# AIRI-Institute/HairFastGAN

Hardware: AMD Instinct MI355X
Metric: stylegan2_generator_fwd_1024_images_per_sec (higher is better)
Workload: dtype f32 tensors + f32 accumulate; conv products as 3 fp16 MFMAs on (hi,lo)-split operands (fp32-class); 1 GPU; StyleGAN2 1024^2 generator forward (range 0->8), random W+, fresh noise per layer, HIP modulated-conv + upfirdn2d kernels (BASELINE.json configs[1]); batch_per_gpu=8, global_batch=8, parallelism=replica x1, weights=synthetic closed-form (oracle/synth.py), conv_precision=f16x3

## Files before the change

### hairfastgan_amd/csrc/convh.hip

```cpp
#define HF_WANT_F16_SPLIT
#include <type_traits>

#include "conv_common.h"

using namespace hf_detail;

#ifdef HF_H_TRACE
__device__ unsigned long long hf_trace_buf[8 * 512];
#define HF_TRACE_POINT(id)                                                                    \
  do {                                                                                         \
    if (blockIdx.x == 0 && blockIdx.y == 0 && lane == 0 && wave < 8 && trace_n < 510) {                    \
      hf_trace_buf[wave * 512 + trace_n++] = ((unsigned long long)(id) << 56) | (__builtin_readcyclecounter() & 0xffffffffffffffULL); \
    }                                                                                          \
  } while (0)
extern "C" int hf_debug_read_trace(unsigned long long *host, int n) {
  return (int)hipMemcpyFromSymbol(host, HIP_SYMBOL(hf_trace_buf), sizeof(unsigned long long) * n);
}
#else
#define HF_TRACE_POINT(id) ((void)0)
#endif

namespace {

typedef _Float16 half8 __attribute__((ext_vector_type(8)));
// ... 2 lines not shown
template <int NR, int NM>
__device__ __forceinline__ void hf_interleave() {
#pragma unroll
  for (int k = 0; k < NR; ++k) {
    __builtin_amdgcn_sched_group_barrier(0x008, 1, 0);
    __builtin_amdgcn_sched_group_barrier(0x100, 1, 0);
  }
  if constexpr (NM > NR) __builtin_amdgcn_sched_group_barrier(0x008, NM - NR, 0);
}

template <int PT, bool UP, int TWMAX, bool FUSE = false>
constexpr int halo_pixels_max() {
  constexpr int h = UP ? 1 : 2;
  constexpr int narrow = (PT / 32 + h) * (32 + h), wide = (PT / TWMAX + h) * (TWMAX + h);
  constexpr int main_tile = wide > narrow ? wide : narrow;
  constexpr int rim = PT >= 512 ? 4 : 2;
  constexpr int rim_tile = (rim + 1) * (PT / rim + 1);
  return (UP && !FUSE && rim_tile > main_tile) ? rim_tile : main_tile;
}

template <bool UP>
__host__ __device__ constexpr int tap_at(int i) {
  return !UP ? i : (i == 2 ? 3 : i == 3 ? 4 : i == 4 ? 2 : i);
}
template <bool UP>
__host__ __device__ constexpr int tap_group(int i) {
  return !UP ? i : (i < 4 ? 0 : i < 6 ? 1 : i < 8 ? 2 : 3);
}
template <bool UP>
__host__ __device__ constexpr int group_first(int g) {
  return !UP ? g : (g == 0 ? 0 : g == 1 ? 4 : g == 2 ? 6 : g == 3 ? 8 : 9);
}

template <int NTERMS, int CT_TILES, int PG, int WAVES_CO, int WAVES_PX, bool UP, int TWMAX, bool FUSE>
struct HShape {
  static constexpr int NW = WAVES_CO * WAVES_PX;
  static constexpr int NT = 64 * NW;
  static constexpr int CT = 32 * CT_TILES * WAVES_CO;
  static constexpr int PT = 32 * PG * WAVES_PX;
  static constexpr int XSLOTS = (PG == 1) ? 4 : 6;
  using Stage = StageLayout<NTERMS, CT, halo_pixels_max<PT, UP, TWMAX, FUSE>(), FUSE ? NW * XSLOTS * 64 : 0>;
  static constexpr int TABLE_FLOATS = 2 * 3 * CT;
  static size_t lds_bytes(int cin, bool rgb) {
    return Stage::stage_bytes + (Stage::cin_table_floats(cin) + (rgb ? 2 : 1) * TABLE_FLOATS) * sizeof(float);
  }
};

template <int NTERMS, int CT_TILES, int PG, int WAVES_CO, int WAVES_PX, bool MOD, bool UP, int TWMAX, bool PRE, bool FUSE = false>
__global__ __launch_bounds__(64 * WAVES_CO * WAVES_PX, (WAVES_CO * WAVES_PX >= 16 ? 4 : 2)) void conv_mfma_h(const ConvParams P,
                                                                          const _Float16 *__restrict__ wth,
                                                                          const _Float16 *__restrict__ wtl) {
  using S = HShape<NTERMS, CT_TILES, PG, WAVES_CO, WAVES_PX, UP, TWMAX, FUSE>;
  using L = typename S::Stage;
  constexpr int NW = S::NW, NT = S::NT, CT = S::CT, PT = S::PT, XSLOTS = S::XSLOTS;
  constexpr int NPH = UP ? 4 : 1;
  constexpr int HALO = UP ? 1 : 2;
  constexpr int NPIX = L::NPIX, NPART = L::NPART, W_UNITS = L::W_UNITS, X_UNITS = L::X_UNITS, BUF_UNITS = L::BUF_UNITS;
  constexpr int N_WPIECE = NPART * W_UNITS / 64;
  constexpr bool PP = PRE && NW == 8;
  constexpr int ND = (N_WPIECE + NW - 1) / NW;
  constexpr int DMA_PER_STEP = PRE ? 1 : (ND + 2) / 3;
  constexpr int XE = (X_UNITS + NT - 1) / NT;
  static_assert(W_UNITS % 64 == 0, "weight part must be whole 1 KiB pieces");
  static_assert(!FUSE || (UP && CT_TILES == 1 && WAVES_CO == 1 && TWMAX == 32), "FUSE: 32 co x (PG*WAVES_PX rows of 32 positions)");
  static_assert(!FUSE || BUF_UNITS * 16 >= NW * XSLOTS * 64 * 16, "FUSE: the exchange of one channel quad must fit a stage buffer");
  static_assert(!PRE || (ND <= 9 && XE <= 8), "PRE issue schedule: one weight DMA per tap-step, activations in odd steps (or every step)");

  HF_DYN_LDS;
  half8 *lds = reinterpret_cast<half8 *>(hf_dyn_lds);
  constexpr int OFF_WL = L::OFF_WL, OFF_XH = L::OFF_XH, OFF_XL = L::OFF_XL;

  const int tid = threadIdx.x;
  const int lane = tid & 63;
  const int wave = tid >> 6;
  const int li = lane & 31;
  const int lh = lane >> 5;
  const int wave_co = (wave / WAVES_PX) * (32 * CT_TILES);
  const int wave_pg = (wave % WAVES_PX) * PG;
  const int blk_x = P.swap_xy ? (int)blockIdx.y : (int)blockIdx.x, blk_y = P.swap_xy ? (int)blockIdx.x : (int)blockIdx.y;
  const int grid_x = P.swap_xy ? (int)gridDim.y : (int)gridDim.x, grid_y = P.swap_xy ? (int)gridDim.x : (int)gridDim.y;
  const int co0 = blk_y * CT;

  const long long plane = (long long)P.h * P.w;
  const int iplane = (int)plane;
  const int nchunks = P.cin / KH;
  float *sl_base = reinterpret_cast<float *>(lds + 2 * BUF_UNITS);
  float *ep_base = sl_base + L::cin_table_floats(P.cin);
  float *rgbw_base = ep_base + S::TABLE_FLOATS;

  struct Tile {
    int gi, b0, ty0, tx0;
  };
  const TileGeom G0 = P.g[0], G1 = P.g[1], G2 = P.g[2];
  auto geom = [&](int gi) {
    TileGeom G;
#define HF_PICK(f) G.f = gi == 0 ? G0.f : (gi == 1 ? G1.f : G2.f)
    HF_PICK(y0); HF_PICK(x0); HF_PICK(dh); HF_PICK(dw); HF_PICK(lg_tw); HF_PICK(lg_th); HF_PICK(lg_nb);
    HF_PICK(tiles_x); HF_PICK(tiles_y); HF_PICK(tiles_b); HF_PICK(first_block);
#undef HF_PICK
    return G;
  };
  auto locate = [&](int t) {
    Tile T;
    T.gi = 0;
    if (P.n_geom > 1 && t >= G1.first_block) T.gi = 1;
    if (P.n_geom > 2 && t >= G2.first_block) T.gi = 2;
    const TileGeom G = geom(T.gi);
    int r = t - G.first_block;
    const int tx = r % G.tiles_x;
    r /= G.tiles_x;
    const int ty = r % G.tiles_y;
    T.b0 = r / G.tiles_y;
    T.ty0 = G.y0 + (ty << G.lg_th);
    T.tx0 = G.x0 + (tx << G.lg_tw);
    if (FUSE) {
      T.ty0 = ty * ((1 << G.lg_th) - 2) - 1;
      T.tx0 = tx * ((1 << G.lg_tw) - 2) - 1;
    }
    return T;
  };
  constexpr int NSRC = XE;
  auto locate_items = [&](const Tile &T, int (&src)[NSRC]) {
    const TileGeom G = geom(T.gi);
    const int wp = (1 << G.lg_tw) + HALO, xs = ((1 << G.lg_th) + HALO) * wp;
#pragma unroll
    for (int e = 0; e < XE; ++e) {
      const int i = tid + e * NT;
      const int kg = i / NPIX, pix = i - kg * NPIX;
      src[e] = -2;
      if (i < X_UNITS && pix < xs) {
        const int hy = pix / wp, hx = pix - hy * wp;
        const int ys = T.ty0 + hy - 1, xc = T.tx0 + hx - 1;
        src[e] = (ys >= 0 && ys < P.h && xc >= 0 && xc < P.w) ? ys * P.w + xc : -1;
      }
    }
  };
  const float w_unscale = *reinterpret_cast<const float *>(wth + 9LL * P.cin * P.cout);
  const bool fast_ep = !UP && HF_STD_STYLED_TAIL(P);
  const float ep_fold = (FUSE || fast_ep) ? P.scale : 1.0f;
  auto load_s = [&](int b, int slot) {
    float *dst = sl_base + slot * P.cin;
    if (MOD)
      for (int i = tid; i < P.cin; i += NT) dst[i] = P.s[(long long)b * P.s_bstride + i];
    float *ep = ep_base + slot * 3 * CT;
    for (int i = tid; i < CT; i += NT) {
      ep[i] = (P.d ? P.d[(long long)b * P.d_bstride + co0 + i] : 1.0f) * w_unscale * ep_fold;
      ep[CT + i] = P.bias ? P.bias[co0 + i] * ep_fold : 0.0f;
      ep[2 * CT + i] = ((!UP || FUSE) && P.oh && P.s_next) ? P.s_next[(long long)b * P.cout + co0 + i] : 1.0f;
    }
    if (!UP && P.rgb_out) {
      float *rw = rgbw_base + slot * 3 * CT;
      for (int i = tid; i < CT; i += NT) {
        const float sv = P.rgb_s[(long long)b * P.cout + co0 + i];
#pragma unroll
        for (int c = 0; c < 3; ++c) rw[c * CT + i] = P.rgb_w[(co0 + i) * 3 + c] * sv;
      }
    }
  };

  int e_src[XE];
  const float *xb;
  int sl_off;
  int sl_slot = 0;

  const unsigned lds_addr0 = hf_lds_addr(lds);
  auto dma_piece = [&](int i, int chunk, int bufsel) {
    const int pc = wave + i * NW;
    if (wave < NW && pc < N_WPIECE) {
      const int part = pc / (W_UNITS / 64), q = pc % (W_UNITS / 64);
      const int u = q * 64 + lane;
      const int row = u / CT, col = u % CT;
      int off = (row * P.cout + co0 + col) * 16;
      HF_OPAQUE_I32(off);
      const _Float16 *src = (part ? wtl : wth) + (long long)chunk * 18 * P.cout * 8;
      hf_glds16_raw_s(src, (unsigned)off, lds_addr0 + (unsigned)(bufsel * BUF_UNITS + part * W_UNITS + q * 64) * 16u);
    }
  };

  const char *xh_b = nullptr, *xl_b = nullptr;
  auto dma_x = [&](int e, int chunk, int bufsel) {
    const int i = tid + e * NT;
    const int kg = i / NPIX;
    const bool inside = e_src[e] >= 0;
    int off = inside ? (kg * iplane + e_src[e]) * 16 : 0;
    HF_OPAQUE_I32(off);
    const long long cofs = (long long)chunk * 2 * plane * 16;
    const unsigned dst = lds_addr0 + (unsigned)(bufsel * BUF_UNITS + OFF_XH + (i - lane)) * 16u;
    hf_glds16_raw_s_if(inside, xh_b + cofs, (unsigned)off, dst);
    if (NTERMS == 3) hf_glds16_raw_s_if(inside, xl_b + cofs, (unsigned)off, dst + (unsigned)X_UNITS * 16u);
    if (e_src[e] == -1) {
      half8 z;
#pragma unroll
      for (int k = 0; k < 8; ++k) z[k] = (_Float16)0.0f;
      half8 *buf = lds + bufsel * BUF_UNITS;
      buf[OFF_XH + i] = z;
      if (NTERMS == 3) buf[OFF_XL + i] = z;
    }
  };

  float xr[XE][8];
  auto load_item = [&](int e, int chunk) {
    const char *xc = reinterpret_cast<const char *>(xb + (long long)chunk * KH * plane);
    const int kg = (tid + e * NT) / NPIX;
    int off = (e_src[e] >= 0) ? kg * 8 * iplane + e_src[e] : 0;
    HF_OPAQUE_I32(off);
#pragma unroll
    for (int k = 0; k < 8; ++k)
      xr[e][k] = *reinterpret_cast<const float *>(xc + (unsigned)((off + k * iplane) * 4));
  };
  auto convert_item = [&](int e, int chunk, half8 *buf) {
    if (e_src[e] == -2) return;
    const int i = tid + e * NT;
    const int kg = i / NPIX;
    half8 hi, lo;
    bool ovf = false;
#pragma unroll
    for (int k = 0; k < 8; ++k) {
      float v = (e_src[e] >= 0) ? xr[e][k] : 0.0f;
      if (MOD) v *= sl_base[sl_off + chunk * KH + kg * 8 + k];
      _Float16 hv, lv;
      hf_split_f16(v, hv, lv, ovf);
      hi[k] = hv;
      lo[k] = lv;
    }
    hf_note_overflow(ovf);
    buf[OFF_XH + i] = hi;
    if (NTERMS == 3) buf[OFF_XL + i] = lo;
  };

  f32x16 acc[NPH][CT_TILES][PG];
  auto zero_acc = [&]() {
#pragma unroll
    for (int ph = 0; ph < NPH; ++ph)
#pragma unroll
      for (int ct = 0; ct < CT_TILES; ++ct)
#pragma unroll
        for (int g = 0; g < PG; ++g)
#pragma unroll
          for (int r = 0; r < 16; ++r) acc[ph][ct][g][r] = 0.0f;
  };
  zero_acc();

  int t_cur = blk_x;
  Tile cur = locate(t_cur);
  locate_items(cur, e_src);
  xb = P.x + (long long)cur.b0 * P.cin * plane;
  if (PRE) {
    xh_b = static_cast<const char *>(P.xh) + (long long)cur.b0 * (P.cin / 8) * plane * 16;
    xl_b = static_cast<const char *>(P.xl) + (long long)cur.b0 * (P.cin / 8) * plane * 16;
  }
  sl_off = 0;
  load_s(cur.b0, 0);
  int ep_slot = 0;
  __syncthreads();
#pragma unroll
  for (int i = 0; i < ND; ++i) dma_piece(i, 0, 0);
  if (PRE) {
#pragma unroll
    for (int e = 0; e < XE; ++e) dma_x(e, 0, 0);
  } else {
#pragma unroll
    for (int e = 0; e < XE; ++e) load_item(e, 0);
#pragma unroll
    for (int e = 0; e < XE; ++e) convert_item(e, 0, lds);
  }
  hf_barrier_keep_young<0>();

  int trace_n = 0;
  (void)trace_n;
  const float nw_ = (!UP && P.noise) ? P.noise_w[0] : 0.0f;
  auto epilogue = [&](const TileGeom &G, const Tile &T, int slot, const float (&nz)[PG]) {
    int co_w = wave_co, li_o = li, lh_o = lh;
    HF_OPAQUE_I32(co_w);
    HF_OPAQUE_I32(li_o);
    HF_OPAQUE_I32(lh_o);
    const int tw = 1 << G.lg_tw, th = 1 << G.lg_th;
    const float *ep = ep_base + slot * 3 * CT;
    const unsigned oplane4 = (unsigned)(P.out_h * P.out_w) * 4u;
    char *ob0 = reinterpret_cast<char *>(P.out + ((long long)T.b0 * P.cout + co0) * ((long long)P.out_h * P.out_w));
#pragma unroll
    for (int g = 0; g < PG; ++g) {
      const int p = (wave_pg + g) * 32 + li_o;
      const int Y = T.ty0 + ((p >> G.lg_tw) & (th - 1)), X = T.tx0 + (p & (tw - 1));
      const bool pv = (Y < G.y0 + G.dh) && (X < G.x0 + G.dw);
      const float nzv = nw_ * nz[g];
      float rgb[3] = {0.0f, 0.0f, 0.0f};
      if (pv) {
      const unsigned pix4 = UP ? (unsigned)(2 * Y * P.out_w + 2 * X) * 4u : (unsigned)(Y * P.out_w + X) * 4u;
#pragma unroll
      for (int ct = 0; ct < CT_TILES; ++ct)
#pragma unroll
        for (int q = 0; q < 4; ++q) {
          const int c4 = co_w + ct * 32 + 8 * q + 4 * lh_o;
          const float4 dm = *reinterpret_cast<const float4 *>(ep + c4);
          const float4 bs = *reinterpret_cast<const float4 *>(ep + CT + c4);
          const float dmv[4] = {dm.x, dm.y, dm.z, dm.w}, bsv[4] = {bs.x, bs.y, bs.z, bs.w};
          unsigned off = (unsigned)c4 * oplane4 + pix4;
#pragma unroll
          for (int k = 0; k < 4; ++k, off += oplane4) {
// ... 135 lines not shown
            hf_half4 h4, l4;
            bool ovf = false;
            hf_split4_f16(vs, h4, l4, ovf);
            if (pvg[g]) {
              ovf_tile = ovf_tile || ovf;
              const unsigned off = cofs16 + pix16[g];
              *reinterpret_cast<hf_half4 *>(oh_t + off) = h4;
              if (ol_t) *reinterpret_cast<hf_half4 *>(ol_t + off) = l4;
            }
          }
          if (RGB) {
#pragma unroll
            for (int c = 0; c < 3; ++c)
              rgb[g][c] = fmaf(v[3], wv[c].w, fmaf(v[2], wv[c].z, fmaf(v[1], wv[c].y, fmaf(v[0], wv[c].x, rgb[g][c]))));
          }
        }
      }
    if (RGB) {
      const int slabs = grid_y * WAVES_CO, slab = blk_y * WAVES_CO + wave / WAVES_PX;
#pragma unroll
      for (int g = 0; g < PG; ++g)
#pragma unroll
        for (int c = 0; c < 3; ++c) {
          const float sum = rgb[g][c] + __shfl_xor(rgb[g][c], 32, 64);
          if (pvg[g] && lh_o == 0)
            P.rgb_out[(((long long)T.b0 * slabs + slab) * 3 + c) * ((long long)P.out_h * P.out_w) + (long long)Yg[g] * P.out_w + Xg[g]] = sum;
        }
    }
    if (SPLIT) hf_note_overflow(ovf_tile);
  };

  const float kxf[4] = {P.blur_kx[0], P.blur_kx[1], P.blur_kx[2], P.blur_kx[3]};
  const float kyf[4] = {P.blur_ky[0], P.blur_ky[1], P.blur_ky[2], P.blur_ky[3]};
  auto epilogue_fused = [&](auto SPLIT_T, const Tile &T, int slot, const float (&nz)[PG][4], int freebuf) {
    constexpr bool SPLIT = decltype(SPLIT_T)::value;
    bool ovf_tile = false;
    int li_o = li, lh_o = lh;
    HF_OPAQUE_I32(li_o);
    HF_OPAQUE_I32(lh_o);
    const float *ep = ep_base + slot * 3 * CT;
    const int wv = wave;
    float *xch = reinterpret_cast<float *>(lds + freebuf * BUF_UNITS);
    const int row0 = wv * PG;
    const int Y0 = T.ty0 + row0, X = T.tx0 + li_o;
    const float nw_f = (P.noise ? P.noise_w[0] : 0.0f) * P.scale;
    const long long oplane = (long long)(2 * P.h) * (2 * P.w);
    const int pix00 = (2 * Y0) * (2 * P.w) + 2 * X;
    const bool colv = li_o >= 1 && li_o <= 30 && X >= 0 && X < P.w;
    char *oh_b = SPLIT ? static_cast<char *>(P.oh) + ((long long)T.b0 * (P.cout >> 3) + (co0 >> 3)) * oplane * 16 : nullptr;
    char *ol_b = SPLIT ? static_cast<char *>(P.ol) + ((long long)T.b0 * (P.cout >> 3) + (co0 >> 3)) * oplane * 16 : nullptr;
    float *of_b = SPLIT ? nullptr : P.out + ((long long)T.b0 * P.cout + co0) * oplane;
#pragma unroll
    for (int q = 0; q < 4; ++q) {
      __builtin_amdgcn_sched_barrier(0);
      float H[4][PG][4];
#pragma unroll
      for (int pr = 0; pr < 2; ++pr)
#pragma unroll
        for (int g = 0; g < PG; ++g)
#pragma unroll
          for (int k = 0; k < 4; ++k) {
            const float t0 = acc[2 * pr][0][g][4 * q + k], t1 = acc[2 * pr + 1][0][g][4 * q + k];
            const float l1 = hf_lane_up(t1), r0 = hf_lane_down(t0), r1 = hf_lane_down(t1);
            H[2 * pr][g][k] = fmaf(kxf[3], r0, fmaf(kxf[2], t1, fmaf(kxf[1], t0, kxf[0] * l1)));
            H[2 * pr + 1][g][k] = fmaf(kxf[3], r1, fmaf(kxf[2], r0, fmaf(kxf[1], t1, kxf[0] * t0)));
          }
      HF_TRACE_POINT(30);
      float4 *xq = reinterpret_cast<float4 *>(xch);
      float4 *mine = xq + (wv * XSLOTS) * 64 + lane;
#pragma unroll
      for (int ph = 0; ph < 4; ++ph) mine[ph * 64] = make_float4(H[ph][0][0], H[ph][0][1], H[ph][0][2], H[ph][0][3]);
      if (PG > 1) {
#pragma unroll
        for (int pc = 0; pc < 2; ++pc)
          mine[(4 + pc) * 64] = make_float4(H[2 + pc][PG - 1][0], H[2 + pc][PG - 1][1], H[2 + pc][PG - 1][2], H[2 + pc][PG - 1][3]);
      }
      HF_TRACE_POINT(31);
      hf_barrier_lds();
      HF_TRACE_POINT(32);
      const float4 *above = xq + (max(wv - 1, 0) * XSLOTS) * 64 + lane, *below = xq + (min(wv + 1, NW - 1) * XSLOTS) * 64 + lane;
      constexpr int ABOVE_P1 = (PG == 1) ? 2 : 4;
      const int c4 = 8 * q + 4 * lh_o;
#pragma unroll
      for (int g = 0; g < PG; ++g) {
        const int rr = row0 + g, Y = Y0 + g;
        const bool pv = colv && rr >= 1 && rr <= PT / 32 - 2 && Y >= 0 && Y < P.h;
#pragma unroll
        for (int a = 0; a < 2; ++a) {
          typedef unsigned u32x2 __attribute__((ext_vector_type(2)));
          typedef unsigned u32x4 __attribute__((ext_vector_type(4)));
          u32x2 hq[2], lq[2];
          bool ovf_a = false;
#pragma unroll
          for (int pc = 0; pc < 2; ++pc) {
            float hm1[4], h2[4], h3[4];
            if (g == 0 && a == 0) {
              const float4 u = above[(ABOVE_P1 + pc) * 64];
              hm1[0] = u.x; hm1[1] = u.y; hm1[2] = u.z; hm1[3] = u.w;
            }
            if (g == PG - 1) {
              const float4 d0 = below[pc * 64];
              h2[0] = d0.x; h2[1] = d0.y; h2[2] = d0.z; h2[3] = d0.w;
              if (a == 1) {
                const float4 d1 = below[(2 + pc) * 64];
                h3[0] = d1.x; h3[1] = d1.y; h3[2] = d1.z; h3[3] = d1.w;
              }
            }
            const float4 dm = *reinterpret_cast<const float4 *>(ep + c4), bs = *reinterpret_cast<const float4 *>(ep + CT + c4);
            const float dmv[4] = {dm.x, dm.y, dm.z, dm.w}, bsv[4] = {bs.x, bs.y, bs.z, bs.w};
            float v[4];
#pragma unroll
            for (int k = 0; k < 4; ++k) {
              const float h_m1 = (g == 0) ? hm1[k] : H[2 + pc][g == 0 ? 0 : g - 1][k];
// ... 65 lines not shown
#pragma unroll
    for (int g = 0; g < PG; ++g) {
      const int p = (wave_pg + g) * 32 + li;
      const int po = ((p >> G.lg_tw) & (th - 1)) * wp + (p & (tw - 1));
#pragma unroll
      for (int r = 0; r < NROW; ++r) pixrow[g][r] = po + r * wp;
    }
    float nzr[PG];
    float nzf[PG][4];
#pragma unroll
    for (int g = 0; g < PG; ++g) {
      nzr[g] = 0.0f;
#pragma unroll
      for (int k = 0; k < 4; ++k) nzf[g][k] = 0.0f;
    }
    HF_TRACE_POINT(7);
    const int t_next = t_cur + grid_x;
    const bool has_next = t_next < P.n_tiles;
    Tile nxt = cur;
    int nxt_sl_off = sl_off;
    if (has_next) {
      nxt = locate(t_next);
      if (nxt.b0 != cur.b0) {
        hf_barrier_lds();
        sl_slot ^= 1;
        nxt_sl_off = sl_slot * P.cin;
        load_s(nxt.b0, sl_slot);
      }
    }
    HF_TRACE_POINT(8);

    for (int c = 0; c < nchunks; ++c, ++stage) {
      const int cb = stage & 1;
      half8 *buf = lds + cb * BUF_UNITS, *nbuf = lds + (cb ^ 1) * BUF_UNITS;
      const bool last = c + 1 == nchunks;
      const bool more1 = !last || has_next;
      const int cpf = last ? 0 : c + 1;
      if (last && has_next) {
        locate_items(nxt, e_src);
        xb = P.x + (long long)nxt.b0 * P.cin * plane;
        if (PRE) {
          xh_b = static_cast<const char *>(P.xh) + (long long)nxt.b0 * (P.cin / 8) * plane * 16;
          xl_b = static_cast<const char *>(P.xl) + (long long)nxt.b0 * (P.cin / 8) * plane * 16;
        }
        sl_off = nxt_sl_off;
      }
      if (last && !UP && P.noise) {
#pragma unroll
        for (int g = 0; g < PG; ++g) {
          const int p = (wave_pg + g) * 32 + li;
          const int Y = min(cur.ty0 + ((p >> G.lg_tw) & (th - 1)), P.h - 1), X = min(cur.tx0 + (p & (tw - 1)), P.w - 1);
          nzr[g] = P.noise[(long long)cur.b0 * P.noise_bstride + (long long)Y * P.out_w + X];
        }
      }
      if (FUSE && last && P.noise) {
#pragma unroll
        for (int g = 0; g < PG; ++g) {
          const int Y = min(max(cur.ty0 + wave_pg + g, 0), P.h - 1), X = min(max(cur.tx0 + li, 0), P.w - 1);
          const float *np = P.noise + (long long)cur.b0 * P.noise_bstride + (long long)(2 * Y) * (2 * P.w) + 2 * X;
          const float2 n0 = *reinterpret_cast<const float2 *>(np), n1 = *reinterpret_cast<const float2 *>(np + 2 * P.w);
          nzf[g][0] = n0.x; nzf[g][1] = n0.y; nzf[g][2] = n1.x; nzf[g][3] = n1.y;
        }
      }
      const half8 *a_hi = buf + lh * CT + wave_co + li;
      const half8 *b_hi = buf + OFF_XH + lh * NPIX;
      constexpr int NSLOT = (UP && !PRE) ? 1 : 2;
      half8 ah[NSLOT][CT_TILES], al[NSLOT][CT_TILES], bh[NSLOT][PG], bl[NSLOT][PG];
      auto fetch_a = [&](int slot, int tap) {
#pragma unroll
        for (int ct = 0; ct < CT_TILES; ++ct) {
          ah[slot][ct] = a_hi[tap * 2 * CT + ct * 32];
          if (NTERMS == 3) al[slot][ct] = a_hi[OFF_WL + tap * 2 * CT + ct * 32];
        }
      };
      auto fetch_b = [&](int slot, int tap) {
        const int ky = tap / 3, kx = tap % 3;
        const int brow = UP ? (ky == 2 ? 0 : 1) : ky, bcol = UP ? (kx == 2 ? 0 : 1) : kx;
#pragma unroll
        for (int g = 0; g < PG; ++g) {
          bh[slot][g] = b_hi[pixrow[g][brow] + bcol];
          if (NTERMS == 3) bl[slot][g] = b_hi[X_UNITS + pixrow[g][brow] + bcol];
        }
      };
      if (PP && pp_half == 1) {
        if (more1) {
#pragma unroll
          for (int j = 0; j < ND; ++j) dma_piece(j, cpf, cb ^ 1);
#pragma unroll
          for (int e = 0; e < XE; ++e) dma_x(e, cpf, cb ^ 1);
        }
        fetch_a(0, tap_at<UP>(0));
        fetch_b(0, tap_at<UP>(0));
        hf_barrier_lds();
      } else {
        fetch_a(0, tap_at<UP>(0));
        fetch_b(0, tap_at<UP>(0));
      }
#pragma unroll
      for (int i = 0; i < 9; ++i) {
        const int tap = tap_at<UP>(i);
        HF_TRACE_POINT(10 + i);
        const int grp = tap_group<UP>(i);
        const int sa = (NSLOT == 1) ? 0 : (i & 1), sb = (NSLOT == 1) ? 0 : (grp & 1);
        if (NSLOT == 1) {
          if (i > 0) fetch_a(0, tap);
          if (i > 0 && group_first<UP>(grp) == i) fetch_b(0, tap);
        } else {
          const bool nb = group_first<UP>(grp) == i && group_first<UP>(grp + 1) < 9;
          if (i + 1 < 9) fetch_a(sa ^ 1, tap_at<UP>(i + 1));
          if (nb) fetch_b(sb ^ 1, tap_at<UP>(group_first<UP>(grp + 1)));
        }
        if (!PP && more1) {
#pragma unroll
          for (int j = 0; j < ND; ++j)
            if (j / DMA_PER_STEP == i) dma_piece(j, cpf, cb ^ 1);
        }
        if (!PP && PRE && more1) {
#pragma unroll
          for (int e = 0; e < XE; ++e)
            if (i == ((2 * XE <= 9) ? 1 + 2 * e : 1 + e)) dma_x(e, cpf, cb ^ 1);
        }
        if (!PRE && more1 && i == 0) {
// ... 8 lines not shown
        HF_TRACE_POINT(20 + i);
        const int ph = UP ? (((tap / 3) & 1) * 2 + ((tap % 3) & 1)) : 0;
#pragma unroll
        for (int ct = 0; ct < CT_TILES; ++ct)
#pragma unroll
          for (int g = 0; g < PG; ++g)
            acc[ph][ct][g] = __builtin_amdgcn_mfma_f32_32x32x16_f16(ah[sa][ct], bh[sb][g], acc[ph][ct][g], 0, 0, 0);
        if (NTERMS == 3) {
#pragma unroll
          for (int ct = 0; ct < CT_TILES; ++ct)
#pragma unroll
            for (int g = 0; g < PG; ++g)
              acc[ph][ct][g] = __builtin_amdgcn_mfma_f32_32x32x16_f16(ah[sa][ct], bl[sb][g], acc[ph][ct][g], 0, 0, 0);
#pragma unroll
          for (int ct = 0; ct < CT_TILES; ++ct)
#pragma unroll
            for (int g = 0; g < PG; ++g)
              acc[ph][ct][g] = __builtin_amdgcn_mfma_f32_32x32x16_f16(al[sa][ct], bh[sb][g], acc[ph][ct][g], 0, 0, 0);
        }
        if constexpr (ILV) {
          constexpr int NRA = CT_TILES * (NTERMS == 3 ? 2 : 1), NRB = PG * (NTERMS == 3 ? 2 : 1), NM = CT_TILES * PG * NTERMS;
          const bool fb = group_first<UP>(grp) == i && group_first<UP>(grp + 1) < 9;
          if (i + 1 < 9 && fb) hf_interleave<(NRA + NRB < NM ? NRA + NRB : NM), NM>();
          else if (i + 1 < 9) hf_interleave<(NRA < NM ? NRA : NM), NM>();
        }
        __builtin_amdgcn_sched_barrier(0);
      }
      HF_TRACE_POINT(2);
      if (PP && pp_half == 0) {
        hf_barrier_lds();
        if (more1) {
#pragma unroll
          for (int j = 0; j < ND; ++j) dma_piece(j, cpf, cb ^ 1);
#pragma unroll
          for (int e = 0; e < XE; ++e) dma_x(e, cpf, cb ^ 1);
        }
      }
      hf_barrier_keep_young<0>();
      HF_TRACE_POINT(3);
    }

    if (FUSE) {
      if (P.oh) epilogue_fused(std::true_type{}, cur, ep_slot, nzf, ((stage - 1) & 1));
      else epilogue_fused(std::false_type{}, cur, ep_slot, nzf, ((stage - 1) & 1));
    } else {
      bool done = false;
      if constexpr (!UP) {
        if (fast_ep) {
          epilogue_fast(G, cur, ep_slot, nzr);
          done = true;
        }
      }
      if (!done) epilogue(G, cur, ep_slot, nzr);
    }
    HF_TRACE_POINT(4);
    if (!has_next) break;
    zero_acc();
    if (nxt.b0 != cur.b0) ep_slot ^= 1;
    cur = nxt;
    t_cur = t_next;
  }
}

__global__ __launch_bounds__(256) void split_weights_absmax(unsigned int *__restrict__ trailer,
                                                            const float *__restrict__ wt, long long n) {
  float m = 0.0f;
  const long long stride = (long long)gridDim.x * blockDim.x;
  for (long long i = (long long)blockIdx.x * blockDim.x + threadIdx.x; i < n; i += stride) m = fmaxf(m, fabsf(wt[i]));
#pragma unroll
  for (int d = 32; d >= 1; d >>= 1) m = fmaxf(m, __shfl_xor(m, d, 64));
  if ((threadIdx.x & 63) == 0 && __float_as_uint(m) > trailer[1]) atomicMax(trailer + 1, __float_as_uint(m));
}
__global__ void split_weights_clear(unsigned int *trailer) {
  if (threadIdx.x < 4) trailer[threadIdx.x] = 0u;
}
__device__ __forceinline__ int weight_prescale_log2(unsigned int absmax_bits) {
  const int e = (int)((absmax_bits >> 23) & 255u) - 127;
// ... 109 lines not shown
      chunk(s);
      load(s, min(c0 + s + RIM_DEPTH, nchunks - 1));
    }
  }
#pragma unroll
  for (int s = 0; s + 1 < RIM_DEPTH; ++s)
    if (c0 + s < nchunks) chunk(s);

  if (!store_ok) return;
  const long long oplane = (long long)P.out_h * P.out_w;
  float *ob = P.out + ((long long)b * P.cout + co0) * oplane +
              (is_row ? (long long)(2 * h) * P.out_w + 2 * p : (long long)(2 * p) * P.out_w + 2 * w);
  const long long second = is_row ? 1 : P.out_w;
  const bool has_second = !is_row || p < w;
#pragma unroll
  for (int r = 0; r < 16; ++r) {
    float *q = ob + (long long)((r & 3) + 8 * (r >> 2) + 4 * lh) * oplane;
    q[0] = acc0[r] * dmv[r];
    if (has_second) q[second] = acc1[r] * dmv[r];
  }
}

inline long long up_rim_blocks(const ConvParams &P) {
  return (long long)P.batch * (hf_cdiv(P.w + 1, 32) + hf_cdiv(P.h, 32)) * (P.cout / 32);
}
template <int NTERMS>
int launch_up_rim(const ConvParams &P, const _Float16 *wth, const _Float16 *wtl, hipStream_t st) {
  const int row_tiles = hf_cdiv(P.w + 1, 32), col_tiles = hf_cdiv(P.h, 32);
  hipLaunchKernelGGL((conv_up_rim_h<NTERMS>), dim3((unsigned)up_rim_blocks(P)), dim3(64), 0, st, P, wth, wtl, row_tiles,
                     row_tiles + col_tiles);
  return hf_launch_status();
}

template <int NTERMS, int CT_TILES, int PG, int WAVES_CO, int WAVES_PX, bool UP, int TWMAX = 32, bool PRE = false, bool FUSE = false>
int launch_h(ConvParams &P, const _Float16 *wth, const _Float16 *wtl, hipStream_t st) {
  using S = HShape<NTERMS, CT_TILES, PG, WAVES_CO, WAVES_PX, UP, TWMAX, FUSE>;
  constexpr int NT = S::NT, CT = S::CT, PT = S::PT, NPIX = S::Stage::NPIX;
  if (P.cin % KH || P.cout % CT || P.stride != 1 || P.t || P.groups > 1 || P.residual || P.act == ACT_PRELU)
    return HF_E_INVALID;
  if ((long long)P.cin * P.h * P.w >= (1LL << 31)) return HF_E_INVALID;
  if ((long long)CT * P.out_h * P.out_w * 4 >= (1LL << 32)) return HF_E_INVALID;
  P.splits = 1;
  P.n_geom = 1;
  P.g[0] = make_geom(0, 0, P.h, P.w, P.batch, PT, 0);
  if (TWMAX > 32 && P.w >= 64 && P.g[0].lg_nb == 0) {
    const int tw = min(TWMAX, pow2_floor(P.w)), th = PT / tw;
    if (th >= 1 && P.h >= th) {
      P.g[0].lg_tw = ilog2(tw); P.g[0].lg_th = ilog2(th);
      P.g[0].tiles_x = hf_cdiv(P.w, tw); P.g[0].tiles_y = hf_cdiv(P.h, th);
    }
  }
  if (FUSE) {
    constexpr int TH = PT / 32;
    P.g[0].lg_tw = 5; P.g[0].lg_th = ilog2(TH); P.g[0].lg_nb = 0;
    P.g[0].tiles_x = hf_cdiv(P.w, 30); P.g[0].tiles_y = hf_cdiv(P.h, TH - 2); P.g[0].tiles_b = P.batch;
  }
  int nblocks = geom_blocks(P.g[0]);
  const bool rim_kernel = UP && !FUSE && PRE && !(g_h_tune & 32);
  if (rim_kernel && up_rim_blocks(P) >= (1LL << 31)) return HF_E_INVALID;
  if (UP && !FUSE && !rim_kernel) {
    P.n_geom = 3;
    constexpr int RIM = PT >= 512 ? 4 : 2;
    P.g[1] = make_geom(P.h, 0, 1, P.w + 1, P.batch, PT, nblocks, true, RIM);
    nblocks += geom_blocks(P.g[1]);
    P.g[2] = make_geom(0, P.w, P.h, 1, P.batch, PT, nblocks, true, RIM);
    nblocks += geom_blocks(P.g[2]);
  }
  for (int i = 0; i < P.n_geom; ++i) {
    if (P.g[i].lg_nb != 0 || (1 << (P.g[i].lg_tw + P.g[i].lg_th)) != PT) return HF_E_INVALID;
    if (geom_xs(P.g[i], 1, UP ? 1 : 2) > NPIX) return HF_E_INVALID;
  }
  const size_t lds = S::lds_bytes(P.cin, P.rgb_out != nullptr);
  if (P.rgb_out && (UP || !P.rgb_w || !P.rgb_s || (!HF_STD_STYLED_TAIL(P) && (WAVES_CO != 1 || P.cout != CT)) ||
                    P.rgb_slabs != P.cout / (32 * CT_TILES)))
    return HF_E_INVALID;
  if (lds > 160 * 1024) return HF_E_INVALID;
  P.n_tiles = nblocks;
  const int co_tiles = P.cout / CT;
  const int per_cu = (2 * lds <= 160 * 1024) ? 2 : 1;
  int resident = (g_h_blocks > 0 ? g_h_blocks : 256 * per_cu) / co_tiles;
  if (resident < 1) resident = 1;
  const bool walk = P.cin / KH >= 2 && (P.cin / KH <= 8 || g_h_blocks > 0);
  const int gx = (walk && nblocks > resident) ? resident : nblocks;
  dim3 grid(gx, co_tiles);
  if (grid.y > 65535) return HF_E_INVALID;
  P.swap_xy = 0;
  if (co_tiles > 1 && gx <= 65535) {
    const double in_bytes = (double)P.batch * P.cin * P.h * P.w * 4.0, w_bytes = 9.0 * P.cin * P.cout * 4.0;
    if (columns_fastest(in_bytes, in_bytes, w_bytes, co_tiles, nblocks)) {
      P.swap_xy = 1;
      grid = dim3(co_tiles, gx);
    }
  }
  if (PRE) {
    if (!P.xh || (NTERMS == 3 && !P.xl) || P.s || (P.cin & 15)) return HF_E_INVALID;
    if ((long long)2 * P.h * P.w * 16 >= (1LL << 31)) return HF_E_INVALID;
    hipLaunchKernelGGL((conv_mfma_h<NTERMS, CT_TILES, PG, WAVES_CO, WAVES_PX, false, UP, TWMAX, PRE, FUSE>), grid, dim3(NT), lds, st,
                       P, wth, wtl);
  } else if (P.s) {
    hipLaunchKernelGGL((conv_mfma_h<NTERMS, CT_TILES, PG, WAVES_CO, WAVES_PX, true, UP, TWMAX, false, FUSE>), grid, dim3(NT), lds, st,
                       P, wth, wtl);
  } else {
    if (FUSE) return HF_E_INVALID;
    hipLaunchKernelGGL((conv_mfma_h<NTERMS, CT_TILES, PG, WAVES_CO, WAVES_PX, false, UP, TWMAX, false, false>), grid, dim3(NT), lds,
                       st, P, wth, wtl);
  }
  const int rc = hf_launch_status();
  if constexpr (UP && !FUSE && PRE) {
    if (rc == HF_OK && rim_kernel) return launch_up_rim<NTERMS>(P, wth, wtl, st);
  }
  return rc;
}

template <int CT_TILES_, int PG_, int WAVES_CO_, int WAVES_PX_, int TWMAX_ = 32>
struct HForm {
  static constexpr int CT_TILES = CT_TILES_, PG = PG_, WAVES_CO = WAVES_CO_, WAVES_PX = WAVES_PX_, TWMAX = TWMAX_;
};
using HForm63 = HForm<1, 2, 1, 8>;
template <bool UP, bool PRE, class F>
int with_h_form(int cfg, F &&f) {
  if constexpr (UP) {
    if (cfg == 63) return f(HForm63{});
    if (cfg == 61) return f(HForm<1, 2, 2, 4>{});
  } else {
    if (cfg == 55) return f(HForm<1, 2, 1, 8, 128>{});
    if constexpr (!PRE) {
      if (cfg == 56) return f(HForm<1, 2, 1, 8, 64>{});
      if (cfg == 54) return f(HForm<1, 2, 1, 4>{});
    }
    if (cfg == 53) return f(HForm<1, 2, 1, 8>{});
    if (cfg == 52) return f(HForm<2, 2, 1, 8>{});
    if (cfg == 51) return f(HForm<1, 2, 2, 4>{});
  }
  return HF_E_INVALID;
}
template <int NTERMS, bool UP, bool PRE, bool FUSE, class Form>
int launch_tile(Form, ConvParams &P, const _Float16 *h, const _Float16 *l, hipStream_t st) {
  return launch_h<NTERMS, Form::CT_TILES, Form::PG, Form::WAVES_CO, Form::WAVES_PX, UP, Form::TWMAX, PRE, FUSE>(P, h, l, st);
}
template <bool UP, bool PRE>
int launch_form(int cfg, int nterms, ConvParams &P, const _Float16 *h, const _Float16 *l, hipStream_t st) {
  return with_h_form<UP, PRE>(cfg, [&](auto form) {
    return with_nterms(nterms, [&](auto nt) { return launch_tile<decltype(nt)::value, UP, PRE, false>(form, P, h, l, st); });
  });
}

}

namespace hf_detail {

thread_local int g_force_h = 0;
thread_local int g_h_blocks = 0;
thread_local int g_h_tune = 0;
int g_batch_invariant = 0;

int launch_conv_h(ConvParams &P, int nterms, bool up, const void *wth, const void *wtl, hipStream_t st) {
  const _Float16 *h = static_cast<const _Float16 *>(wth), *l = static_cast<const _Float16 *>(wtl);
  if (!h || (nterms == 3 && !l)) return HF_E_INVALID;
  int cfg, rc;
  if (up) {
    cfg = (P.cout % 64) ? 63 : 61;
    rc = P.xh ? launch_form<true, true>(cfg, nterms, P, h, l, st) : launch_form<true, false>(cfg, nterms, P, h, l, st);
    if (rc == HF_OK) note_path(5, P.xh ? cfg + 20 : cfg);
    return rc;
  }
  cfg = g_force_h;
  if (cfg == 0) {
    const long long blocks52 = (long long)P.batch * hf_cdiv(P.h, 16) * hf_cdiv(P.w, 32) * (P.cout / 64);
    if (P.cout % 64) cfg = (P.w >= 128) ? 55 : 53;
    else cfg = (P.h * P.w >= 512 && blocks52 >= 256) ? 52 : 51;
  }
// ... 72 lines not shown
  return launch_conv_h(P, nterms, false, wt_hi, wt_lo, (hipStream_t)stream);
}

extern "C" int hf_modconv3x3_up_f16_f32(float *tmp, const float *x, const void *wt_hi, const void *wt_lo, int nterms,
                                        const float *s, const float *d, int batch, int cin, int cout, int h, int w,
                                        int tmp_pitch, void *stream) {
  ConvParams P{};
  if (!tmp || !x || gen_fill(P, x, nullptr, nullptr, wt_hi, nterms, s, d, batch, cin, cout, h, w, true, tmp_pitch) != HF_OK)
    return HF_E_INVALID;
  P.out = tmp;
  return launch_conv_h(P, nterms, true, wt_hi, wt_lo, (hipStream_t)stream);
}

extern "C" int hf_modconv3x3_up_blur_f16_f32(float *out, void *split_hi, void *split_lo, const float *x, const void *x_hi,
                                             const void *x_lo, const void *wt_hi, const void *wt_lo, const float *s,
                                             const float *d, const float *blur_k1d_x, const float *blur_k1d_y, const float *noise, const float *noise_w,
                                             long long noise_bstride, const float *bias, const float *s_next, int batch, int cin,
                                             int cout, int h, int w, float alpha, float scale, void *stream) {
  const int nterms = wt_lo ? 3 : 1;
  ConvParams P{};
  if (gen_fill(P, x, x_hi, x_lo, wt_hi, nterms, x_hi ? nullptr : s, d, batch, cin, cout, h, w) != HF_OK ||
      gen_tail(P, noise, noise_w, noise_bstride, bias, alpha, scale) != HF_OK || (!out == !split_hi) || !blur_k1d_x ||
      !blur_k1d_y || h < 2 || w < 2 || (!x_hi && !s) || (cout % 32) || (cin % 16) ||
      (split_hi && ((nterms == 3 && !split_lo) || (cout & 7))) || !bias || !(alpha >= 0.0f && alpha <= 1.0f) || !(scale > 0.0f))
    return HF_E_INVALID;
  P.out = out;
  P.out_h = 2 * h; P.out_w = 2 * w; P.out_wv = 2 * w;
  P.oh = split_hi; P.ol = nterms == 3 ? split_lo : nullptr; P.s_next = s_next;
  for (int j = 0; j < 4; ++j) {
    P.blur_kx[j] = blur_k1d_x[3 - j];
    P.blur_ky[j] = blur_k1d_y[3 - j];
  }
  const _Float16 *hi = static_cast<const _Float16 *>(wt_hi), *lo = static_cast<const _Float16 *>(wt_lo);
  const int rc = with_nterms(nterms, [&](auto nt) {
    return x_hi ? launch_tile<decltype(nt)::value, true, true, true>(HForm63{}, P, hi, lo, (hipStream_t)stream)
                : launch_tile<decltype(nt)::value, true, false, true>(HForm63{}, P, hi, lo, (hipStream_t)stream);
  });
  if (rc == HF_OK) note_path(5, x_hi ? 93 : 73);
  return rc;
}

extern "C" int hf_set_batch_invariant(int on) {
  const int prev = hf_detail::g_batch_invariant;
  hf_detail::g_batch_invariant = on ? 1 : 0;
  return prev;
}

extern "C" int hf_debug_set_tuning(int bits) {
  hf_detail::g_h_tune = bits;
  return HF_OK;
}

extern "C" int hf_modconv3x3_f16_rgb_slabs(int cout) {
  return cout <= 0 || (cout % 32) ? 0 : ((cout % 64) ? cout / 32 : cout / 64);
}

extern "C" int hf_debug_set_persistent_blocks(int blocks) {
  hf_detail::g_h_blocks = blocks;
  return HF_OK;
}

extern "C" int hf_modconv3x3_f16_rgb_f32(float *out, const float *x, const void *wt_hi, const void *wt_lo, int nterms,
                                         const float *s, const float *d, const float *noise, const float *noise_w,
                                         long long noise_bstride, const float *bias, int batch, int cin, int cout,
                                         int h, int w, float alpha, float scale, float *rgb_raw, const float *rgb_wt,
                                         const float *rgb_s, void *stream) {
  ConvParams P{};
// ... 56 lines not shown
```

Measured before the change: 1776 images/s.

## Add three-slot activation ring to the fused pre-split upsampling conv

New measurement: 1762 images/s. Within noise of the previous version (-0.8%).

```diff
diff --git a/hairfastgan_amd/csrc/convh.hip b/hairfastgan_amd/csrc/convh.hip
--- a/hairfastgan_amd/csrc/convh.hip
+++ b/hairfastgan_amd/csrc/convh.hip
@@ -58,7 +58,7 @@
   return !UP ? g : (g == 0 ? 0 : g == 1 ? 4 : g == 2 ? 6 : g == 3 ? 8 : 9);
 }
 
-template <int NTERMS, int CT_TILES, int PG, int WAVES_CO, int WAVES_PX, bool UP, int TWMAX, bool FUSE>
+template <int NTERMS, int CT_TILES, int PG, int WAVES_CO, int WAVES_PX, bool UP, int TWMAX, bool FUSE, int XRING = 2>
 struct HShape {
   static constexpr int NW = WAVES_CO * WAVES_PX;
   static constexpr int NT = 64 * NW;
@@ -67,8 +67,13 @@
   static constexpr int XSLOTS = (PG == 1) ? 4 : 6;
   using Stage = StageLayout<NTERMS, CT, halo_pixels_max<PT, UP, TWMAX, FUSE>(), FUSE ? NW * XSLOTS * 64 : 0>;
   static constexpr int TABLE_FLOATS = 2 * 3 * CT;
+  static constexpr int XW_X = 5;
+  static constexpr int WS_UNITS = Stage::NPART * Stage::W_UNITS > (NW - XW_X) * XSLOTS * 64 ? Stage::NPART * Stage::W_UNITS : (NW - XW_X) * XSLOTS * 64;
+  static constexpr int XS_UNITS = Stage::NPART * Stage::X_UNITS > XW_X * XSLOTS * 64 ? Stage::NPART * Stage::X_UNITS : XW_X * XSLOTS * 64;
+  static constexpr int RING_UNITS = 2 * WS_UNITS + 3 * XS_UNITS;
+  static constexpr size_t stage_bytes = XRING == 3 ? (size_t)RING_UNITS * 16 : Stage::stage_bytes;
   static size_t lds_bytes(int cin, bool rgb) {
-    return Stage::stage_bytes + (Stage::cin_table_floats(cin) + (rgb ? 2 : 1) * TABLE_FLOATS) * sizeof(float);
+    return stage_bytes + (Stage::cin_table_floats(cin) + (rgb ? 2 : 1) * TABLE_FLOATS) * sizeof(float);
   }
 };
 
@@ -76,7 +81,8 @@
 __global__ __launch_bounds__(64 * WAVES_CO * WAVES_PX, (WAVES_CO * WAVES_PX >= 16 ? 4 : 2)) void conv_mfma_h(const ConvParams P,
                                                                           const _Float16 *__restrict__ wth,
                                                                           const _Float16 *__restrict__ wtl) {
-  using S = HShape<NTERMS, CT_TILES, PG, WAVES_CO, WAVES_PX, UP, TWMAX, FUSE>;
+  constexpr int XRING = (MOD && PRE) ? 3 : 2;
+  using S = HShape<NTERMS, CT_TILES, PG, WAVES_CO, WAVES_PX, UP, TWMAX, FUSE, XRING>;
   using L = typename S::Stage;
   constexpr int NW = S::NW, NT = S::NT, CT = S::CT, PT = S::PT, XSLOTS = S::XSLOTS;
   constexpr int NPH = UP ? 4 : 1;
@@ -91,10 +97,15 @@
   static_assert(!FUSE || (UP && CT_TILES == 1 && WAVES_CO == 1 && TWMAX == 32), "FUSE: 32 co x (PG*WAVES_PX rows of 32 positions)");
   static_assert(!FUSE || BUF_UNITS * 16 >= NW * XSLOTS * 64 * 16, "FUSE: the exchange of one channel quad must fit a stage buffer");
   static_assert(!PRE || (ND <= 9 && XE <= 8), "PRE issue schedule: one weight DMA per tap-step, activations in odd steps (or every step)");
+  constexpr bool RING3 = XRING == 3;
+  static_assert(XRING == 2 || (RING3 && FUSE && PP), "ring 3: the one-kernel upsampling conv's ping-pong form only");
 
   HF_DYN_LDS;
   half8 *lds = reinterpret_cast<half8 *>(hf_dyn_lds);
   constexpr int OFF_WL = L::OFF_WL, OFF_XH = L::OFF_XH, OFF_XL = L::OFF_XL;
+  constexpr int W_STRIDE = RING3 ? S::WS_UNITS : BUF_UNITS, X_STRIDE = RING3 ? S::XS_UNITS : BUF_UNITS;
+  constexpr int X_BASE = RING3 ? 2 * S::WS_UNITS : OFF_XH;
+  constexpr int STAGE_UNITS = RING3 ? S::RING_UNITS : 2 * BUF_UNITS;
 
   const int tid = threadIdx.x;
   const int lane = tid & 63;
@@ -110,7 +121,7 @@
   const long long plane = (long long)P.h * P.w;
   const int iplane = (int)plane;
   const int nchunks = P.cin / KH;
-  float *sl_base = reinterpret_cast<float *>(lds + 2 * BUF_UNITS);
+  float *sl_base = reinterpret_cast<float *>(lds + STAGE_UNITS);
   float *ep_base = sl_base + L::cin_table_floats(P.cin);
   float *rgbw_base = ep_base + S::TABLE_FLOATS;
 
@@ -166,10 +177,12 @@
   const float ep_fold = (FUSE || fast_ep) ? P.scale : 1.0f;
   auto load_s = [&](int b, int slot) {
     float *dst = sl_base + slot * P.cin;
-    if (MOD)
+    if (MOD && !PRE)
       for (int i = tid; i < P.cin; i += NT) dst[i] = P.s[(long long)b * P.s_bstride + i];
     float *ep = ep_base + slot * 3 * CT;
-    for (int i = tid; i < CT; i += NT) {
+    int t0 = tid;
+    if constexpr (RING3) HF_OPAQUE_I32(t0);
+    for (int i = t0; i < CT; i += NT) {
       ep[i] = (P.d ? P.d[(long long)b * P.d_bstride + co0 + i] : 1.0f) * w_unscale * ep_fold;
       ep[CT + i] = P.bias ? P.bias[co0 + i] * ep_fold : 0.0f;
       ep[2 * CT + i] = ((!UP || FUSE) && P.oh && P.s_next) ? P.s_next[(long long)b * P.cout + co0 + i] : 1.0f;
@@ -199,7 +212,7 @@
       int off = (row * P.cout + co0 + col) * 16;
       HF_OPAQUE_I32(off);
       const _Float16 *src = (part ? wtl : wth) + (long long)chunk * 18 * P.cout * 8;
-      hf_glds16_raw_s(src, (unsigned)off, lds_addr0 + (unsigned)(bufsel * BUF_UNITS + part * W_UNITS + q * 64) * 16u);
+      hf_glds16_raw_s(src, (unsigned)off, lds_addr0 + (unsigned)(bufsel * W_STRIDE + part * W_UNITS + q * 64) * 16u);
     }
   };
 
@@ -211,17 +224,23 @@
     int off = inside ? (kg * iplane + e_src[e]) * 16 : 0;
     HF_OPAQUE_I32(off);
     const long long cofs = (long long)chunk * 2 * plane * 16;
-    const unsigned dst = lds_addr0 + (unsigned)(bufsel * BUF_UNITS + OFF_XH + (i - lane)) * 16u;
+    const unsigned dst = lds_addr0 + (unsigned)(bufsel * X_STRIDE + X_BASE + (i - lane)) * 16u;
     hf_glds16_raw_s_if(inside, xh_b + cofs, (unsigned)off, dst);
     if (NTERMS == 3) hf_glds16_raw_s_if(inside, xl_b + cofs, (unsigned)off, dst + (unsigned)X_UNITS * 16u);
     if (e_src[e] == -1) {
       half8 z;
 #pragma unroll
       for (int k = 0; k < 8; ++k) z[k] = (_Float16)0.0f;
-      half8 *buf = lds + bufsel * BUF_UNITS;
-      buf[OFF_XH + i] = z;
-      if (NTERMS == 3) buf[OFF_XL + i] = z;
-    }
+      half8 *buf = lds + bufsel * X_STRIDE;
+      buf[X_BASE + i] = z;
+      if (NTERMS == 3) buf[X_BASE + X_UNITS + i] = z;
+    }
+  };
+  auto dma_x_count = [&]() {
+    int n = 0;
+#pragma unroll
+    for (int e = 0; e < XE; ++e) n += hf_wave_any(e_src[e] >= 0) ? NPART : 0;
+    return n;
   };
 
   float xr[XE][8];
@@ -279,18 +298,32 @@
   load_s(cur.b0, 0);
   int ep_slot = 0;
   __syncthreads();
+  int xslot = 0, x_young = 0;
+  if constexpr (RING3) x_young = dma_x_count();
+  auto barrier_keep_n = [&](int n) {
+    static_assert(!RING3 || XE <= 3, "barrier_keep_n: one case per count");
+    if (n >= 3 * NPART) hf_barrier_keep_young<3 * NPART>();
+    else if (n >= 2 * NPART) hf_barrier_keep_young<2 * NPART>();
+    else if (n >= NPART) hf_barrier_keep_young<NPART>();
+    else hf_barrier_keep_young<0>();
+  };
 #pragma unroll
   for (int i = 0; i < ND; ++i) dma_piece(i, 0, 0);
   if (PRE) {
 #pragma unroll
     for (int e = 0; e < XE; ++e) dma_x(e, 0, 0);
+    if constexpr (RING3) {
+#pragma unroll
+      for (int e = 0; e < XE; ++e) dma_x(e, 1, 1);
+    }
   } else {
 #pragma unroll
     for (int e = 0; e < XE; ++e) load_item(e, 0);
 #pragma unroll
     for (int e = 0; e < XE; ++e) convert_item(e, 0, lds);
   }
-  hf_barrier_keep_young<0>();
+  if constexpr (RING3) barrier_keep_n(x_young);
+  else hf_barrier_keep_young<0>();
 
   int trace_n = 0;
   (void)trace_n;
@@ -492,7 +525,7 @@
 
   const float kxf[4] = {P.blur_kx[0], P.blur_kx[1], P.blur_kx[2], P.blur_kx[3]};
   const float kyf[4] = {P.blur_ky[0], P.blur_ky[1], P.blur_ky[2], P.blur_ky[3]};
-  auto epilogue_fused = [&](auto SPLIT_T, const Tile &T, int slot, const float (&nz)[PG][4], int freebuf) {
+  auto epilogue_fused = [&](auto SPLIT_T, const Tile &T, int slot, const float (&nz)[PG][4], int freebuf, int freex) {
     constexpr bool SPLIT = decltype(SPLIT_T)::value;
     bool ovf_tile = false;
     int li_o = li, lh_o = lh;
@@ -501,6 +534,14 @@
     const float *ep = ep_base + slot * 3 * CT;
     const int wv = wave;
     float *xch = reinterpret_cast<float *>(lds + freebuf * BUF_UNITS);
+    auto xwave = [&](int v) -> float4 * {
+      if constexpr (RING3) {
+        const int u = v < S::XW_X ? X_BASE + freex * X_STRIDE + v * (XSLOTS * 64) : freebuf * W_STRIDE + (v - S::XW_X) * (XSLOTS * 64);
+        return reinterpret_cast<float4 *>(lds) + u + lane;
+      } else {
+        return reinterpret_cast<float4 *>(xch) + (v * XSLOTS) * 64 + lane;
+      }
+    };
     const int row0 = wv * PG;
     const int Y0 = T.ty0 + row0, X = T.tx0 + li_o;
     const float nw_f = (P.noise ? P.noise_w[0] : 0.0f) * P.scale;
@@ -526,8 +567,7 @@
             H[2 * pr + 1][g][k] = fmaf(kxf[3], r1, fmaf(kxf[2], r0, fmaf(kxf[1], t1, kxf[0] * t0)));
           }
       HF_TRACE_POINT(30);
-      float4 *xq = reinterpret_cast<float4 *>(xch);
-      float4 *mine = xq + (wv * XSLOTS) * 64 + lane;
+      float4 *mine = xwave(wv);
 #pragma unroll
       for (int ph = 0; ph < 4; ++ph) mine[ph * 64] = make_float4(H[ph][0][0], H[ph][0][1], H[ph][0][2], H[ph][0][3]);
       if (PG > 1) {
@@ -538,7 +578,7 @@
       HF_TRACE_POINT(31);
       hf_barrier_lds();
       HF_TRACE_POINT(32);
-      const float4 *above = xq + (max(wv - 1, 0) * XSLOTS) * 64 + lane, *below = xq + (min(wv + 1, NW - 1) * XSLOTS) * 64 + lane;
+      const float4 *above = xwave(max(wv - 1, 0)), *below = xwave(min(wv + 1, NW - 1));
       constexpr int ABOVE_P1 = (PG == 1) ? 2 : 4;
       const int c4 = 8 * q + 4 * lh_o;
 #pragma unroll
@@ -670,12 +710,17 @@
 
     for (int c = 0; c < nchunks; ++c, ++stage) {
       const int cb = stage & 1;
-      half8 *buf = lds + cb * BUF_UNITS, *nbuf = lds + (cb ^ 1) * BUF_UNITS;
+      half8 *buf = lds + cb * W_STRIDE, *nbuf = lds + (cb ^ 1) * BUF_UNITS;
       const bool last = c + 1 == nchunks;
       const bool more1 = !last || has_next;
       const int cpf = last ? 0 : c + 1;
-      if (last && has_next) {
+      const bool xwrap = c + 2 >= nchunks;
+      const bool more2 = !xwrap || has_next;
+      const int cpx = xwrap ? c + 2 - nchunks : c + 2;
+      const int xs2 = xslot == 0 ? 2 : xslot - 1;
+      if ((RING3 ? c + 2 == nchunks : last) && has_next) {
         locate_items(nxt, e_src);
+        if constexpr (RING3) x_young = dma_x_count();
         xb = P.x + (long long)nxt.b0 * P.cin * plane;
         if (PRE) {
           xh_b = static_cast<const char *>(P.xh) + (long long)nxt.b0 * (P.cin / 8) * plane * 16;
@@ -701,7 +746,7 @@
         }
       }
       const half8 *a_hi = buf + lh * CT + wave_co + li;
-      const half8 *b_hi = buf + OFF_XH + lh * NPIX;
+      const half8 *b_hi = (RING3 ? lds + xslot * X_STRIDE : buf) + X_BASE + lh * NPIX;
       constexpr int NSLOT = (UP && !PRE) ? 1 : 2;
       half8 ah[NSLOT][CT_TILES], al[NSLOT][CT_TILES], bh[NSLOT][PG], bl[NSLOT][PG];
       auto fetch_a = [&](int slot, int tap) {
@@ -724,8 +769,16 @@
         if (more1) {
 #pragma unroll
           for (int j = 0; j < ND; ++j) dma_piece(j, cpf, cb ^ 1);
-#pragma unroll
-          for (int e = 0; e < XE; ++e) dma_x(e, cpf, cb ^ 1);
+          if constexpr (!RING3) {
+#pragma unroll
+            for (int e = 0; e < XE; ++e) dma_x(e, cpf, cb ^ 1);
+          }
+        }
+        if constexpr (RING3) {
+          if (more2) {
+#pragma unroll
+            for (int e = 0; e < XE; ++e) dma_x(e, cpx, xs2);
+          }
         }
         fetch_a(0, tap_at<UP>(0));
         fetch_b(0, tap_at<UP>(0));
@@ -800,17 +853,30 @@
         if (more1) {
 #pragma unroll
           for (int j = 0; j < ND; ++j) dma_piece(j, cpf, cb ^ 1);
-#pragma unroll
-          for (int e = 0; e < XE; ++e) dma_x(e, cpf, cb ^ 1);
-        }
-      }
-      hf_barrier_keep_young<0>();
+          if constexpr (!RING3) {
+#pragma unroll
+            for (int e = 0; e < XE; ++e) dma_x(e, cpf, cb ^ 1);
+          }
+        }
+        if constexpr (RING3) {
+          if (more2) {
+#pragma unroll
+            for (int e = 0; e < XE; ++e) dma_x(e, cpx, xs2);
+          }
+        }
+      }
+      if constexpr (RING3) {
+        barrier_keep_n(more2 ? x_young : 0);
+        xslot = xslot == 2 ? 0 : xslot + 1;
+      } else {
+        hf_barrier_keep_young<0>();
+      }
       HF_TRACE_POINT(3);
     }
 
     if (FUSE) {
-      if (P.oh) epilogue_fused(std::true_type{}, cur, ep_slot, nzf, ((stage - 1) & 1));
-      else epilogue_fused(std::false_type{}, cur, ep_slot, nzf, ((stage - 1) & 1));
+      if (P.oh) epilogue_fused(std::true_type{}, cur, ep_slot, nzf, ((stage - 1) & 1), xslot == 0 ? 2 : xslot - 1);
+      else epilogue_fused(std::false_type{}, cur, ep_slot, nzf, ((stage - 1) & 1), xslot == 0 ? 2 : xslot - 1);
     } else {
       bool done = false;
       if constexpr (!UP) {
@@ -986,12 +1052,16 @@
   return hf_launch_status();
 }
 
-template <int NTERMS, int CT_TILES, int PG, int WAVES_CO, int WAVES_PX, bool UP, int TWMAX = 32, bool PRE = false, bool FUSE = false>
+template <int NTERMS, int CT_TILES, int PG, int WAVES_CO, int WAVES_PX, bool UP, int TWMAX = 32, bool PRE = false, bool FUSE = false,
+          int XRING = 2>
 int launch_h(ConvParams &P, const _Float16 *wth, const _Float16 *wtl, hipStream_t st) {
-  using S = HShape<NTERMS, CT_TILES, PG, WAVES_CO, WAVES_PX, UP, TWMAX, FUSE>;
+  using S = HShape<NTERMS, CT_TILES, PG, WAVES_CO, WAVES_PX, UP, TWMAX, FUSE, XRING>;
   constexpr int NT = S::NT, CT = S::CT, PT = S::PT, NPIX = S::Stage::NPIX;
+  static_assert(XRING == 2 || (XRING == 3 && FUSE && PRE && CT_TILES == 1 && PG == 2 && WAVES_CO == 1 && WAVES_PX == 8),
+                "ring 3: the pre-split one-kernel upsampling conv in the shape of HForm63");
   if (P.cin % KH || P.cout % CT || P.stride != 1 || P.t || P.groups > 1 || P.residual || P.act == ACT_PRELU)
     return HF_E_INVALID;
+  if (XRING == 3 && P.cin / KH < 2) return HF_E_INVALID;
   if ((long long)P.cin * P.h * P.w >= (1LL << 31)) return HF_E_INVALID;
   if ((long long)CT * P.out_h * P.out_w * 4 >= (1LL << 32)) return HF_E_INVALID;
   P.splits = 1;
@@ -1049,8 +1119,8 @@
   if (PRE) {
     if (!P.xh || (NTERMS == 3 && !P.xl) || P.s || (P.cin & 15)) return HF_E_INVALID;
     if ((long long)2 * P.h * P.w * 16 >= (1LL << 31)) return HF_E_INVALID;
-    hipLaunchKernelGGL((conv_mfma_h<NTERMS, CT_TILES, PG, WAVES_CO, WAVES_PX, false, UP, TWMAX, PRE, FUSE>), grid, dim3(NT), lds, st,
-                       P, wth, wtl);
+    hipLaunchKernelGGL((conv_mfma_h<NTERMS, CT_TILES, PG, WAVES_CO, WAVES_PX, XRING == 3, UP, TWMAX, PRE, FUSE>), grid, dim3(NT), lds,
+                       st, P, wth, wtl);
   } else if (P.s) {
     hipLaunchKernelGGL((conv_mfma_h<NTERMS, CT_TILES, PG, WAVES_CO, WAVES_PX, true, UP, TWMAX, false, FUSE>), grid, dim3(NT), lds, st,
                        P, wth, wtl);
@@ -1088,9 +1158,9 @@
   }
   return HF_E_INVALID;
 }
-template <int NTERMS, bool UP, bool PRE, bool FUSE, class Form>
+template <int NTERMS, bool UP, bool PRE, bool FUSE, int XRING = 2, class Form>
 int launch_tile(Form, ConvParams &P, const _Float16 *h, const _Float16 *l, hipStream_t st) {
-  return launch_h<NTERMS, Form::CT_TILES, Form::PG, Form::WAVES_CO, Form::WAVES_PX, UP, Form::TWMAX, PRE, FUSE>(P, h, l, st);
+  return launch_h<NTERMS, Form::CT_TILES, Form::PG, Form::WAVES_CO, Form::WAVES_PX, UP, Form::TWMAX, PRE, FUSE, XRING>(P, h, l, st);
 }
 template <bool UP, bool PRE>
 int launch_form(int cfg, int nterms, ConvParams &P, const _Float16 *h, const _Float16 *l, hipStream_t st) {
@@ -1229,7 +1299,9 @@
     P.blur_ky[j] = blur_k1d_y[3 - j];
   }
   const _Float16 *hi = static_cast<const _Float16 *>(wt_hi), *lo = static_cast<const _Float16 *>(wt_lo);
+  const bool ring3 = x_hi && !(g_h_tune & 64) && cin / KH >= 2;
   const int rc = with_nterms(nterms, [&](auto nt) {
+    if (ring3) return launch_tile<decltype(nt)::value, true, true, true, 3>(HForm63{}, P, hi, lo, (hipStream_t)stream);
     return x_hi ? launch_tile<decltype(nt)::value, true, true, true>(HForm63{}, P, hi, lo, (hipStream_t)stream)
                 : launch_tile<decltype(nt)::value, true, false, true>(HForm63{}, P, hi, lo, (hipStream_t)stream);
   });
```
